# ktncktnc/diffusion-forcing-transformer

Hardware: AMD Instinct MI355X
Metric: denoised latent frames/sec, DFoT RE10K 8f & 200f rollout @1/2/4/8 GPU (higher is better)
Workload: dtype bf16

## Files before the change

diffusion-forcing-transformer_amd/backbone.py:

```python
from __future__ import annotations

import ctypes as C
import math
from typing import Dict, Optional, Sequence, Tuple

import torch
from torch import nn

from . import capi, ops


def _get(cfg, key, default=None):
    if isinstance(cfg, dict):
        return cfg.get(key, default)
    return getattr(cfg, key, default) if not hasattr(cfg, "get") else cfg.get(key, default)


class _Node(nn.Module):
    """Anonymous container so that dotted reference key names map onto a module tree."""


class UViT3DPose(nn.Module):
    def __init__(self, cfg, x_shape: Sequence[int], max_tokens: int, external_cond_dim: int = 0,
                 external_cond_type: str = "action", external_cond_num_classes: Optional[int] = None,
# ... 42 lines not shown
            self._register(name, tuple(shape[k] for k in range(ndim.value)))
            self._names.append(name)
        self._synced: Optional[Tuple] = None
        self._reserved = 0
        self._op_key: Optional[int] = None
        self._cond_key = None
        self._cond_refs = None
        self._cond_gen = None
        self._cond_flag = None
        self.cond_cache_stats = {"builds": 0, "identity_hits": 0, "content_hits": 0}
        self._train_names = None
        self._trainer = None
        self._trainer_sig = None
        self.live_frames = None
        self.fresh_frames = None
        self._fresh_key = None
        self._train_stamp = 0
        self._dropout_generator: Optional[torch.Generator] = None

    def _register(self, name: str, shape: Tuple[int, ...]) -> None:
        *path, leaf = name.split(".")
        node: nn.Module = self
        for part in path:
            if part not in node._modules:
                node.add_module(part, _Node())
            node = node._modules[part]
        t = torch.zeros(shape, dtype=torch.float32)
        if name in self._persistent_buffers:
            node.register_buffer(leaf, t, persistent=True)
        else:
# ... 228 lines not shown
            self._cond_refs = (external_cond, external_cond_mask)
            self._cond_gen = self.reserve_generation
        out = torch.empty_like(xf)
        live = self.live_frames
        if live is not None:
            if tuple(live.shape) != (b, self.temporal_length) or live.dtype != torch.uint8 or not live.is_contiguous():
                raise ValueError(f"live_frames must be a contiguous uint8 tensor of shape {(b, self.temporal_length)}")
            capi.require_device(dev, live_frames=live)
        fresh = self.fresh_frames
        if fresh is not None:
            if tuple(fresh.shape) != (b, self.temporal_length) or fresh.dtype != torch.uint8 or not fresh.is_contiguous():
                raise ValueError(f"fresh_frames must be a contiguous uint8 tensor of shape {(b, self.temporal_length)}")
            capi.require_device(dev, fresh_frames=fresh)
            if key != self._fresh_key:
                fresh = None
        capi.check(capi.lib.dfot_uvit_forward_cached_masks(self._handle, capi.ptr(xf, torch.float32, "x"),
                                                           capi.ptr(kf, torch.float32, "noise_levels"), capi.ptr(out), b,
                                                           capi.ptr(live, torch.uint8, "live_frames"),
                                                           capi.ptr(fresh, torch.uint8, "fresh_frames"), capi.stream_ptr()))
        self._fresh_key = key
        return out.to(x.dtype)

    def read_tap(self, name: str, channels: int, level: int, batch: int) -> torch.Tensor:
        r = self.x_shape[-1] // 2 // (2 ** level)
        out = torch.empty(batch * self.temporal_length, channels, r, r, device="cuda", dtype=torch.float32)
        capi.check(capi.lib.dfot_uvit_read_tap(self._handle, name.encode(), capi.ptr(out), out.numel(), capi.stream_ptr()))
        return out

    def __del__(self):
        try:
            if getattr(self, "_handle", None) and self._handle.value:
                capi.lib.dfot_uvit_destroy(self._handle)
                self._handle = C.c_void_p()
        except Exception:
# ... 2 lines not shown
```

diffusion-forcing-transformer_amd/capi.py:

```python
from __future__ import annotations

import ctypes as C
import os

_HERE = os.path.dirname(os.path.abspath(__file__))
LIB_PATH = os.environ.get("DFOT_LIB", os.path.join(_HERE, "libdfot_hip.so"))

OK, ERR_ARG, ERR_SHAPE, ERR_HIP, ERR_STATE, ERR_NAME = range(6)


class DfotError(RuntimeError):
    def __init__(self, code: int, message: str):
        super().__init__(f"libdfot_hip error {code}: {message}")
        self.code = code


class UViTConfig(C.Structure):
    _fields_ = [
        ("channels", C.c_int32 * 4), ("emb_channels", C.c_int32), ("num_updown_blocks", C.c_int32 * 3),
        ("num_mid_blocks", C.c_int32), ("num_heads", C.c_int32), ("in_channels", C.c_int32),
        ("resolution", C.c_int32), ("max_tokens", C.c_int32), ("cond_dim", C.c_int32), ("noise_dim", C.c_int32),
        ("rope_theta", C.c_float), ("eps", C.c_float),
    ]

# ... 53 lines not shown
    "dfot_uvit_num_params": (_I, [_P]),
    "dfot_uvit_param_name": (C.c_char_p, [_P, _I]),
    "dfot_uvit_param_shape": (_I, [_P, _I, C.POINTER(_L), C.POINTER(_I)]),
    "dfot_uvit_load_weight": (_I, [_P, C.c_char_p, _P, C.POINTER(_L), _I, _P]),
    "dfot_uvit_finalize": (_I, [_P, _P]),
    "dfot_uvit_reserve": (_I, [_P, _I]),
    "dfot_uvit_workspace_bytes": (C.c_size_t, [_P]),
    "dfot_uvit_set_option": (_I, [_P, C.c_char_p, _I]),
    "dfot_uvit_query": (_I, [_P, C.c_char_p, C.POINTER(C.c_double)]),
    "dfot_uvit_attn_timing": (_I, [_P, C.POINTER(C.c_double), C.POINTER(_L)]),
    "dfot_uvit_forward": (_I, [_P, _P, _P, _P, _P, _P, _I, _P]),
    "dfot_uvit_set_conditions": (_I, [_P, _P, _P, _I, _P]),
    "dfot_uvit_forward_cached": (_I, [_P, _P, _P, _P, _I, _P]),
    "dfot_uvit_forward_cached_live": (_I, [_P, _P, _P, _P, _I, _P, _P]),
    "dfot_uvit_forward_cached_masks": (_I, [_P, _P, _P, _P, _I, _P, _P, _P]),
    "dfot_uvit_read_tap": (_I, [_P, C.c_char_p, _P, C.c_size_t, _P]),
    "dfot_uvit3d_create": (_I, [C.POINTER(UViT3DConfig), C.POINTER(_P)]),
    "dfot_uvit3d_config_bytes": (_L, []),
    "dfot_uvit3d_forward": (_I, [_P, _P, _P, _P, _P, _P, _I, _P]),
    "dfot_uvit3d_forward_live": (_I, [_P, _P, _P, _P, _P, _P, _I, _P, _P]),
    "dfot_op_gn_film_silu": (_I, [_P, _P, _P, _P, _P, _P, _P, _P, _I, _I, _I, _I, _P]),
    "dfot_op_rms_film": (_I, [_P, _P, _P, _P, _P, _P, _L, _I, _I, _I, _F, _P]),
    "dfot_dit_create": (_I, [C.POINTER(DiTConfig), C.POINTER(_P)]),
    "dfot_dit_create_f": (_I, [C.POINTER(DiTConfigF), C.POINTER(_P)]),
    "dfot_dit_destroy": (_I, [_P]),
    "dfot_dit_num_params": (_I, [_P]),
    "dfot_dit_param_name": (C.c_char_p, [_P, _I]),
    "dfot_dit_param_shape": (_I, [_P, _I, C.POINTER(_L), C.POINTER(_I)]),
    "dfot_dit_load_weight": (_I, [_P, C.c_char_p, _P, C.POINTER(_L), _I, _P]),
    "dfot_dit_finalize": (_I, [_P, _P]),
# ... 163 lines not shown
```

diffusion-forcing-transformer_amd/csrc/kernels.h:

```cpp
#pragma once
#include "common.h"

namespace dfot {

int launch_noise_emb(const float* k, const float* freqs, const float* phases, const float* w1, const float* b1,
                     const float* w2, const float* b2, float* hidden, float* out, int bt, int ndim, int e, hipStream_t s);
int launch_uvit3d_emb(const float* k, const float* freqs, const float* phases, const float* w1, const float* b1, const float* w2,
                      const float* b2, const float* cond, const uint8_t* cond_mask, const float* a_w1, const float* a_b1,
                      const float* a_w2, const float* a_b2, float* out, int bt, int ndim, int cdim, int e, int tokens, hipStream_t s);
int launch_embed_input(const float* x, const float* w, const float* b, float* out, int bt, int res, int cin, int c0,
                       hipStream_t s);
int launch_cond_repack(const float* cond, bf16* a, int bt, int res, int cdim, int kpad, hipStream_t s);
int launch_emb_pyramid(const bf16* emb0, bf16* emb1, bf16* emb2, bf16* emb3, int bt, int r0, int e, hipStream_t s);
int launch_project_output(const float* x0, const float* w, const float* b, float* out, int bt, int res, int c0, int cout,
                          hipStream_t s, const uint8_t* live = nullptr);
int launch_gn_partial_f32(const float* x, float* partial, int bt, int pixels, int c, hipStream_t s);
int launch_gn_partial_bf16(const bf16* x, float* partial, int bt, int pixels, int c, hipStream_t s);
int launch_gn_finalize(const float* partial, float* stats, int bt, int nblk, int pixels, int c, float eps, hipStream_t s);
int gn_partial_blocks(int pixels);
int launch_gn_apply_silu(const float* x, const float* stats, const float* gamma, const float* beta, bf16* out, int bt,
                         int pixels, int c, hipStream_t s, const uint8_t* live = nullptr);
struct FilmChunk {
  const bf16* w;
  const float* b;
// ... 42 lines not shown
                    int img_w = 0, int sdy = 0, int sdx = 0, int all_taps = 0);
struct WgradPlan {
  int form, slices;
};
WgradPlan wgrad_plan(int m, int n, long rows, long max_slices);
int launch_wgrad_conv_taps(const bf16* dy, const bf16* x, float* out, int co, int ci, long pix, int slices, int img_h, int img_w, hipStream_t s);
int wgrad_conv_tiles(int co, int ci, int* target);
int launch_wgrad_nt_plan(const bf16* a, long lda, const bf16* b, long ldb, float* out, int m, int n, long rows, WgradPlan plan, hipStream_t s);
int launch_vloss_grad(const float* x, const float* noise, const float* v, const float* a, const float* sg, const float* coef, float* dv,
                      int batch, int tokens, long f, bool vspace, hipStream_t s);
int launch_sumsq(const float* x, long n, float* out, hipStream_t s);
int launch_adamw(float* p, const float* g, float* m, float* v, long n, float lr, float b1, float b2, float eps, float wd, int step,
                 const float* sumsq, float max_norm, float* ema, float ema_decay, hipStream_t s);
int launch_f32_to_bf16(const float* src, bf16* dst, long n, hipStream_t s);
int launch_bf16_to_f32(const bf16* src, float* dst, long n, hipStream_t s);
int launch_equal_bits(const void* a, const void* b, long bytes, int* differs, hipStream_t s);
int launch_pack_rows(const float* src, bf16* dst, const int* map, int rows, int k, int kpad, long ldd, int col0,
                     hipStream_t s);
int launch_pack_conv3(const float* src, bf16* dst, int co, int ci, hipStream_t s);
int launch_gather_f32(const float* src, float* dst, const int* map, int n, hipStream_t s);
int launch_nhwc_to_nchw(const float* src, float* dst, int bt, int p, int c, hipStream_t s);
int launch_bf16_nhwc_to_nchw(const bf16* src, float* dst, int bt, int p, int c, hipStream_t s);

struct AttnScratch {
  float* p = nullptr;
  size_t bytes = 0;
};
int launch_attention(const bf16* q, const bf16* k, const bf16* v, bf16* o, long ldo, int batch, int heads, int n, int d,
                     int variant, hipStream_t stream, AttnScratch* scratch = nullptr);
int launch_attention_v3(const bf16* q, const bf16* k, const bf16* v, bf16* o, long ldo, int batch, int heads, int n, bool nomax,
// ... 31 lines not shown
```

diffusion-forcing-transformer_amd/csrc/kernels.hip:

```cpp
#include "kernels.h"
#include "dfot_hip.h"

namespace dfot {

typedef __attribute__((ext_vector_type(4))) float float4v;
typedef __attribute__((ext_vector_type(2))) float float2v;

__device__ __forceinline__ float wave_sum(float v) {
#pragma unroll
  for (int o = 32; o > 0; o >>= 1) v += __shfl_xor(v, o);
  return v;
}

template <bool FOURIER>
__global__ __launch_bounds__(256) void noise_mlp_kernel(const float* __restrict__ in, const float* __restrict__ freqs,
                                                        const float* __restrict__ phases, const float* __restrict__ w,
                                                        const float* __restrict__ b, float* __restrict__ out, int kdim,
                                                        int e) {
  const int lane = threadIdx.x & 63, wave = threadIdx.x >> 6;
  const int row = blockIdx.x * 4 + wave;
  const int bt = blockIdx.y;
  if (row >= e) return;
  float acc = 0.f;
  for (int i = lane; i < kdim; i += 64) {
// ... 1293 lines not shown
  const bf16x8 v = reinterpret_cast<const bf16x8*>(s)[i];
  float4v a, b;
#pragma unroll
  for (int j = 0; j < 4; ++j) a[j] = bf2f(v[j]), b[j] = bf2f(v[4 + j]);
  reinterpret_cast<float4v*>(d)[2 * i] = a;
  reinterpret_cast<float4v*>(d)[2 * i + 1] = b;
}
static bool aligned16(const void* a, const void* b) { return (((uintptr_t)a | (uintptr_t)b) & 15) == 0; }
int launch_f32_to_bf16(const float* src, bf16* dst, long n, hipStream_t s) {
  const long n8 = aligned16(src, dst) ? n / 8 : 0;
  if (n8) hipLaunchKernelGGL(f32_to_bf16_kernel8, dim3(cdiv(n8, 256)), dim3(256), 0, s, src, dst, n8);
  if (n - 8 * n8) hipLaunchKernelGGL(f32_to_bf16_kernel, dim3(cdiv(n - 8 * n8, 256)), dim3(256), 0, s, src + 8 * n8, dst + 8 * n8, n - 8 * n8);
  DFOT_CHECK_HIP(hipGetLastError());
  return DFOT_OK;
}
int launch_bf16_to_f32(const bf16* src, float* dst, long n, hipStream_t s) {
  const long n8 = aligned16(src, dst) ? n / 8 : 0;
  if (n8) hipLaunchKernelGGL(bf16_to_f32_kernel8, dim3(cdiv(n8, 256)), dim3(256), 0, s, src, dst, n8);
  if (n - 8 * n8) hipLaunchKernelGGL(bf16_to_f32_kernel, dim3(cdiv(n - 8 * n8, 256)), dim3(256), 0, s, src + 8 * n8, dst + 8 * n8, n - 8 * n8);
  DFOT_CHECK_HIP(hipGetLastError());
  return DFOT_OK;
}

__global__ void pack_rows_kernel(const float* __restrict__ src, bf16* __restrict__ dst, const int* __restrict__ map, long total,
                                 int k, int kpad, long ldd, int col0) {
  const long i = (long)blockIdx.x * blockDim.x + threadIdx.x;
  if (i >= total) return;
  const int kk = (int)(i % kpad);
  const long r = i / kpad;
  const long sr = map ? map[r] : r;
// ... 207 lines not shown
```

diffusion-forcing-transformer_amd/csrc/uvit.hip:

```cpp
#include <algorithm>
#include <cmath>
#include <cstdarg>
#include <cstdlib>
#include <cstring>
#include <functional>
#include <map>
#include <string>
#include <vector>

#include "dfot_hip.h"
#include "gemm.h"
#include "kernels.h"

namespace dfot {

static thread_local char g_err[1024] = "";
void set_error(const char* fmt, ...) {
  va_list ap;
  va_start(ap, fmt);
  vsnprintf(g_err, sizeof(g_err), fmt, ap);
  va_end(ap);
}
const char* get_error() { return g_err; }

// ... 71 lines not shown
  int film_chunks = 0;
  uint8_t* cond_mask = nullptr;
  bool have_mask = false;
  int cond_batch = 0;
  int64_t cond_builds = 0;
  bf16 *acond = nullptr, *emb[4] = {nullptr, nullptr, nullptr, nullptr}, *s1 = nullptr, *hbf = nullptr,
       *cat = nullptr, *q = nullptr, *k = nullptr, *v = nullptr;
  AttnScratch attn_scratch;
  const float* pend_part = nullptr;
  float* out_part = nullptr;
  size_t out_part_elems = 0;
  const float* pend_bias = nullptr;
  int pend_lvl = 0, pend_c = 0, pend_slices = 2;
  long pend_m = 0;
  int last_batch = 0;
  const float* xin[4] = {nullptr, nullptr, nullptr, nullptr};
  bf16* XB[4] = {nullptr, nullptr, nullptr, nullptr};
  bool xin_bf[4] = {false, false, false, false};
  int gemm_variant = GEMM_AUTO;
  int attn_variant = 2;
  bool attn_force_safe = false;
  bool time_attn = false;
  std::vector<hipEvent_t> ev_start, ev_stop;
  size_t ev_used = 0;
};

namespace dfot {

template <typename T>
static int dev_alloc(dfot_uvit_s* h, T** out, size_t count, bool workspace = false) {
// ... 428 lines not shown
  g.A = h->s1; g.W = h->up_conv[l].w; g.M = bt * rr * rr; g.N = cout; g.K = 9 * cin; g.H = rr; g.Wd = rr; g.Cin = cin;
  g.zeros = h->zeros; g.bias = h->up_conv[l].b; g.out_f32 = h->tmp; g.ldo = cout;
  if (live && (rr * rr) % 256 == 0 && h->gemm_variant == GEMM_AUTO) g.live = live;
  if ((rc = conv_between_levels(h, g, s))) return rc;
  h->gn1_nblk = 0;
  if (!h->xin_bf[l]) {
    set_error("run_up: level %d stream is not in its bf16 buffer", l);
    return DFOT_ERR_STATE;
  }
  return launch_upsample_add_bf16(h->tmp, h->XB[l], h->XB[l], bt, rr, rr, cout, s, live);
}

}

static int forward_from_emb(dfot_uvit_s* h, const float* x, float* out, int batch, const uint8_t* live_frames, const uint8_t* fresh_frames,
                            hipStream_t s);

extern "C" {

const char* dfot_last_error(void) { return get_error(); }
int dfot_version(void) { return 1; }

int dfot_uvit_create(const dfot_uvit_config* cfg, dfot_uvit_t* out) {
  DFOT_REQUIRE(cfg && out, DFOT_ERR_ARG, "dfot_uvit_create: null argument");
  DFOT_REQUIRE(cfg->resolution % 16 == 0 && cfg->resolution >= 32, DFOT_ERR_SHAPE, "resolution %d must be a multiple of 16", cfg->resolution);
  DFOT_REQUIRE(cfg->emb_channels % 64 == 0, DFOT_ERR_SHAPE, "emb_channels %d must be a multiple of 64", cfg->emb_channels);
  DFOT_REQUIRE(cfg->in_channels <= 3 && cfg->cond_dim % 20 == 0, DFOT_ERR_SHAPE, "in_channels %d / cond_dim %d unsupported", cfg->in_channels, cfg->cond_dim);
  for (int l = 0; l < 4; ++l)
    DFOT_REQUIRE(cfg->channels[l] % 64 == 0, DFOT_ERR_SHAPE, "channels[%d]=%d must be a multiple of 64", l, cfg->channels[l]);
  DFOT_REQUIRE(cfg->channels[0] % 128 == 0 && cfg->channels[1] % 128 == 0, DFOT_ERR_SHAPE, "ResBlock channels must be multiples of 128");
  for (int l = 2; l < 4; ++l) {
// ... 180 lines not shown
      sv_off += (long)bt * 2 * c;
      return DFOT_OK;
    };
    for (int l = 0; l < 2; ++l) {
      for (ResW& w : h->down_res[l]) if ((rc = add(&w.fcache, &w.sv_off, w.w_film, w.b_film, w.c, l))) return rc;
      for (ResW& w : h->up_res[l]) if ((rc = add(&w.fcache, &w.sv_off, w.w_film, w.b_film, w.c, l))) return rc;
    }
    for (TrW& w : h->down_tr) if ((rc = add(&w.fcache, &w.sv_off, w.w_film, w.b_film, w.c, 2))) return rc;
    for (TrW& w : h->up_tr) if ((rc = add(&w.fcache, &w.sv_off, w.w_film, w.b_film, w.c, 2))) return rc;
    for (TrW& w : h->mid_tr) if ((rc = add(&w.fcache, &w.sv_off, w.w_film, w.b_film, w.c, 3))) return rc;
    if ((rc = dev_alloc(h, &h->sv, (size_t)sv_off, true))) return rc;
    if ((rc = dev_alloc(h, &h->film_table, table.size(), true))) return rc;
    DFOT_CHECK_HIP(hipMemcpy(h->film_table, table.data(), table.size() * sizeof(FilmChunk), hipMemcpyHostToDevice));
    h->film_chunks = (int)table.size();
    if ((rc = dev_alloc(h, &h->cond_mask, (size_t)max_batch, true))) return rc;
    h->cond_batch = 0;
  }
  if ((rc = dev_alloc(h, &h->cat, mc * 5, true))) return rc;
  if ((rc = dev_alloc(h, &h->q, mc, true))) return rc;
  if ((rc = dev_alloc(h, &h->k, mc, true))) return rc;
  if ((rc = dev_alloc(h, &h->v, mc, true))) return rc;
  {
    const size_t e2 = bt * pix[2] * h->ch[2], e3 = bt * pix[3] * h->ch[3];
    h->out_part_elems = 3 * (e2 > e3 ? e2 : e3);
    if ((rc = dev_alloc(h, &h->out_part, h->out_part_elems, true))) return rc;
  }
  {
    size_t need = 16;
    for (int b = 1; b <= max_batch; ++b)
      for (int l = 2; l < 4; ++l) need = std::max(need, attention_scratch_bytes(b, h->heads, h->T * h->r[l] * h->r[l], h->ch[l] / h->heads));
// ... 41 lines not shown
    set_error("set_option: unknown key '%s'", key);
    return DFOT_ERR_ARG;
  }
  return DFOT_OK;
}

int dfot_uvit_query(dfot_uvit_t h, const char* key, double* value) {
  DFOT_REQUIRE(h && key && value, DFOT_ERR_ARG, "query: null argument");
  DFOT_REQUIRE(h->finalized, DFOT_ERR_STATE, "query: weights not finalized");
  float bound = 0.f;
  for (const TrW& w : h->down_tr) bound = fmaxf(bound, w.score_bound);
  for (const TrW& w : h->up_tr) bound = fmaxf(bound, w.score_bound);
  if (!strcmp(key, "score_bound_l2")) *value = bound;
  else if (!strcmp(key, "attn_kernel_l2")) *value = (bound < 64.0f && !h->attn_force_safe) ? 14 : 5;
  else if (!strcmp(key, "cond_builds")) *value = (double)h->cond_builds;
  else {
    set_error("query: unknown key '%s'", key);
    return DFOT_ERR_ARG;
  }
  return DFOT_OK;
}

int dfot_uvit_set_conditions(dfot_uvit_t h, const float* external_cond, const uint8_t* external_cond_mask, int batch,
                             void* stream) {
  DFOT_REQUIRE(h, DFOT_ERR_ARG, "set_conditions: null handle");
  DFOT_REQUIRE(!h->posefree, DFOT_ERR_STATE, "set_conditions: a pose-free handle (dfot_uvit3d_create) has no pose caches; call dfot_uvit3d_forward");
  DFOT_REQUIRE(external_cond != nullptr, DFOT_ERR_ARG, "External condition (camera pose) is required for U-ViT3DPose model.");
  DFOT_REQUIRE(h->finalized, DFOT_ERR_STATE, "set_conditions: weights not finalized");
  DFOT_REQUIRE(batch > 0 && batch <= h->max_batch, DFOT_ERR_STATE, "set_conditions: batch %d exceeds reserved %d", batch, h->max_batch);
  hipStream_t s = (hipStream_t)stream;
// ... 28 lines not shown
  h->cond_batch = batch;
  return DFOT_OK;
}

int dfot_uvit_forward_cached(dfot_uvit_t h, const float* x, const float* noise_levels, float* out, int batch, void* stream) {
  return dfot_uvit_forward_cached_live(h, x, noise_levels, out, batch, nullptr, stream);
}

int dfot_uvit_forward_cached_live(dfot_uvit_t h, const float* x, const float* noise_levels, float* out, int batch, const uint8_t* live_frames,
                                  void* stream) {
  return dfot_uvit_forward_cached_masks(h, x, noise_levels, out, batch, live_frames, nullptr, stream);
}

int dfot_uvit_forward_cached_masks(dfot_uvit_t h, const float* x, const float* noise_levels, float* out, int batch, const uint8_t* live_frames,
                                   const uint8_t* fresh_frames, void* stream) {
  DFOT_REQUIRE(h && x && noise_levels && out, DFOT_ERR_ARG, "forward: null argument");
  DFOT_REQUIRE(!fresh_frames || h->last_batch == batch, DFOT_ERR_STATE,
               "forward: frozen frames need the previous forward of this handle to have run the same batch (%d, now %d)", h->last_batch, batch);
  DFOT_REQUIRE(!fresh_frames || live_frames, DFOT_ERR_ARG, "forward: frozen frames must also be dead frames (live_frames is null)");
  DFOT_REQUIRE(!h->posefree, DFOT_ERR_STATE, "forward_cached: a pose-free handle (dfot_uvit3d_create) runs through dfot_uvit3d_forward");
  DFOT_REQUIRE(h->finalized, DFOT_ERR_STATE, "forward: weights not finalized");
  DFOT_REQUIRE(batch > 0 && batch == h->cond_batch, DFOT_ERR_STATE,
               "forward_cached: batch %d does not match the cached conditions (%d)", batch, h->cond_batch);
  hipStream_t s = (hipStream_t)stream;
  const dfot_uvit_config& c = h->cfg;
  const int bt = batch * h->T, e = h->E;
  int rc = 0;
  if ((rc = launch_noise_emb(noise_levels, h->ne_freqs, h->ne_phases, h->ne_w1, h->ne_b1, h->ne_w2, h->ne_b2, h->nhid,
                             h->nemb, bt, c.noise_dim, e, s)))
    return rc;
  return forward_from_emb(h, x, out, batch, live_frames, fresh_frames, s);
}

}

static int forward_from_emb(dfot_uvit_s* h, const float* x, float* out, int batch, const uint8_t* live_frames, const uint8_t* fresh_frames,
                            hipStream_t s) {
  const dfot_uvit_config& c = h->cfg;
  const int bt = batch * h->T, e = h->E;
  int rc = 0;
  if ((rc = launch_film_vec(h->film_table, h->film_chunks, h->nemb, h->sv, bt, e, s))) return rc;
  if ((rc = launch_embed_input_bf16(x, h->ein_w, h->ein_b, h->XB[0], bt, c.resolution, c.in_channels, h->ch[0], s))) return rc;
  h->gn1_nblk = 0;
  for (int l = 0; l < 4; ++l) h->xin[l] = h->X[l];
  h->xin_bf[0] = true;
  h->xin_bf[1] = h->xin_bf[2] = h->xin_bf[3] = false;

  if (fresh_frames && (h->gemm_variant != GEMM_AUTO || (h->r[2] * h->r[2]) % 512 != 0)) fresh_frames = nullptr;
  for (int l = 0; l < 2; ++l) {
    for (const ResW& w : h->down_res[l])
      if ((rc = run_res_block(h, w, l, bt, s, fresh_frames))) return rc;
    if ((rc = run_down(h, l, bt, s, fresh_frames))) return rc;
  }
  h->pend_bias = nullptr;
  for (const TrW& w : h->down_tr)
    if ((rc = run_tr_block(h, w, 2, batch, s))) return rc;
  if ((rc = flush_pending(h, s))) return rc;
  if ((rc = run_down(h, 2, bt, s))) return rc;
  for (const TrW& w : h->mid_tr)
    if ((rc = run_tr_block(h, w, 3, batch, s))) return rc;
  if ((rc = flush_pending(h, s))) return rc;
  if ((rc = run_up(h, 2, bt, s))) return rc;
  for (const TrW& w : h->up_tr)
    if ((rc = run_tr_block(h, w, 2, batch, s))) return rc;
  if ((rc = flush_pending(h, s))) return rc;
  for (int l = 1; l >= 0; --l) {
    if ((rc = run_up(h, l, bt, s, live_frames))) return rc;
// ... 211 lines not shown
```

diffusion-forcing-transformer_amd/sampler.py:

```python
from __future__ import annotations

from dataclasses import dataclass, field
from typing import Callable, Dict, List, Optional, Tuple

import numpy as np
import torch

from . import capi, parallel
from .diffusion import DiffusionConfig, Schedule
from .guidance import HistoryGuidance


@dataclass
class SamplerConfig:
    x_shape: Tuple[int, int, int] = (3, 256, 256)
    max_tokens: int = 8
    diffusion: DiffusionConfig = field(default_factory=DiffusionConfig)
    scheduling_matrix: str = "full_sequence"
    is_full_sequence: bool = False
    prediction_guidance: Dict = field(default_factory=lambda: {"name": "conditional"})
    interpolation_guidance: Dict = field(default_factory=lambda: {"name": "conditional"})
    keyframe_density: Optional[float] = None
    sliding_context_len: Optional[int] = None
    interpolation_max_batch_size: Optional[int] = None
# ... 21 lines not shown
        self.schedule = Schedule(cfg.diffusion)
        self.noise_fn = noise_fn or device_noise_fn(clip=cfg.diffusion.clip_noise)
        self.timesteps = cfg.diffusion.timesteps
        self.sampling_timesteps = cfg.diffusion.sampling_timesteps
        self.max_tokens = cfg.max_tokens
        self.x_shape = tuple(cfg.x_shape)
        self.trace: List[dict] = []
        self.window_forwards = 0
        self.shard_windows = False
        self.branch_parallel = False
        self._branch_split_active = False
        self.device = "cuda"
        self.dry_run = False
        self.use_graph = True
        self.skip_frozen_frames = True
        self.skip_dead_frames = True
        self.graph_replays = 0
        self.graph_captures = 0
        self._graphs: Dict[tuple, dict] = {}
        self._graphs_generation = 0
        if cfg.diffusion.sampling_timesteps > cfg.diffusion.timesteps:
            raise ValueError("sampling_timesteps must be <= timesteps")

    @torch.no_grad()
    def _process_conditions(self, conditions: Optional[torch.Tensor], noise_levels=None) -> Optional[torch.Tensor]:
        if conditions is None:
            return None
        if conditions.shape[-1] != 16:
            raise ValueError(f"raw camera poses must have 16 values per frame, got {conditions.shape[-1]}")
        cfg = self.cfg
# ... 187 lines not shown
            qb = np.where(repl, qb_c, np.float32(0)).astype(np.float32)
            excl = None
            if plan.excluded is not None:
                excl = plan.excluded.reshape(bm, horizon)
                qa, qb = np.where(excl, np.float32(0), qa), np.where(excl, np.float32(1), qb)
            sa, s1, an, cn, keepf, sigma = sch.ddim_coef(lv, tl) if sch.is_ddim_sampling else sch.ddpm_coef(lv)
            sigma = np.where(keepf != 0, np.float32(0), sigma).astype(np.float32)
            tables = np.stack([qa, qb, sa, s1, an, cn, keepf, sch.model_level(lv)]).astype(np.float32)
            plans.append(dict(plan=plan, nfe=plan.nfe, bm=bm, need_noise=bool(repl.any()) or excl is not None, excl=excl, tables=tables,
                              sigma=sigma if bool((sigma != 0).any()) else None,
                              gen=(mask == 0).astype(np.uint8),
                              cmask=None if plan.cond_masked is None else np.tile(plan.cond_masked, batch_size)))
        if not plans:
            return (xs[:, :-padding] if padding > 0 else xs), None
        strict = bool(getattr(self.noise_fn, "strict_order", False))

        def draw_noise(p_):
            nfe, bm, need = p_["nfe"], p_["bm"], p_["need_noise"]
            noise = None
            if history_guidance.is_simple:
                if nfe == 2 and (need or strict):
                    drawn = self.noise_fn("q_sample", (batch_size, horizon, *x_shape))
                    noise = torch.zeros(batch_size, 2, horizon, *x_shape, device=dev, dtype=torch.float32)
                    noise[:, 0] = drawn.to(device=dev, dtype=torch.float32)
            else:
                g = p_["plan"].n_gen
                bh = bm // g
                if need or strict:
                    noise = self.noise_fn("q_sample", (bh, horizon, *x_shape)).to(device=dev, dtype=torch.float32)
                    if g > 1:
# ... 70 lines not shown
                for p_ in plans:
                    if p_.get("renoise"):
                        continue
                    lv = p_["plan"].levels.reshape(p_["bm"], horizon)
                    key = (lv == self.timesteps - 1).tobytes() + bytes([p_["nfe"]])
                    if key not in by_mask:
                        by_mask[key] = self._process_conditions(conditions.repeat_interleave(p_["nfe"], dim=0), lv)
                    p_["cond"] = by_mask[key]
            finally:
                self._interpolate_masked_poses = False
        fresh_dev = torch.from_numpy(np.concatenate([a.ravel() for a in self._fresh_flags(plans, batch_size, horizon)])).cuda()
        foff = 0
        for p_ in plans:
            p_["fresh_dev"] = fresh_dev[foff:foff + p_["bm"] * horizon].view(p_["bm"], horizon)
            foff += p_["bm"] * horizon
        xs = xs.contiguous()
        s = capi.stream_ptr
        branch_cache: Dict[tuple, tuple] = {}

        skip_dead = self.skip_dead_frames and hasattr(self.model, "live_frames")
        skip_frozen = skip_dead and self.skip_frozen_frames and hasattr(self.model, "fresh_frames")

        def step(p_, xs, noise, tables, gen_dev, xs_next=None, live_dev=None, fresh_dev=None):
            nonlocal cond_rep, cond_nfe
            nfe, bm = p_["nfe"], p_["bm"]
            x_in = torch.empty(bm, horizon, *x_shape, device="cuda", dtype=torch.float32)
            capi.check(capi.lib.dfot_hg_prepare(capi.ptr(xs), capi.ptr(noise), capi.ptr(tables[0]), capi.ptr(tables[1]),
                                                capi.ptr(x_in), batch_size, nfe, horizon, f, s()))
            if cond_full is not None and cond_nfe != nfe:
                cond_rep = cond_full if nfe == 1 else cond_full.repeat_interleave(nfe, dim=0)
                cond_nfe = nfe
            if "cond" in p_:
                cond_rep = p_["cond"]
            lvl = tables[7] if cfg.diffusion.is_continuous else tables[7].to(torch.int32)
            world, rank = parallel.world_info()
            if nfe in split_nfe:
                hb = rank % nfe
                key = (id(cond_rep), id(p_["cmask_dev"]), hb)
# ... 7 lines not shown
                if skip_dead:
                    self.model.live_frames = gen_dev
                try:
                    v = parallel.exchange_branches(self.model(x_h, l_h, c_h, m_h), nfe)
                    self.branch_exchanges = getattr(self, "branch_exchanges", 0) + 1
                finally:
                    if skip_dead:
                        self.model.live_frames = None
            elif rg > 0:
                v = self._reconstruction_guided_v(x_in, lvl, cond_rep, p_["cmask_dev"], tables, gen_dev, rg_ctx, rg, nfe)
            else:
                if skip_dead:
                    self.model.live_frames = live_dev if live_dev is not None else p_["live_dev"]
                if skip_frozen:
                    self.model.fresh_frames = fresh_dev if fresh_dev is not None else p_["fresh_dev"]
                try:
                    v = self.model(x_in, lvl, cond_rep, p_["cmask_dev"])
                finally:
                    if skip_dead:
                        self.model.live_frames = None
                    if skip_frozen:
                        self.model.fresh_frames = None
            step_noise = None
            if strict or p_["sigma"] is not None:
                step_noise = self.noise_fn("ddim", (bm, horizon, *x_shape))
            if xs_next is None:
                xs_next = torch.empty_like(xs)
            compose = capi.lib.dfot_ddim_compose_tokw if p_["tokw"] else capi.lib.dfot_ddim_compose
            capi.check(compose(capi.ptr(xs), capi.ptr(x_in), capi.ptr(v), capi.ptr(tables[2]),
                                                  capi.ptr(tables[3]), capi.ptr(tables[4]), capi.ptr(tables[5]),
                                                  capi.ptr(tables[6]), capi.ptr(p_["weights_dev"]), capi.ptr(gen_dev),
                                                  capi.ptr(xs_next), batch_size, nfe, horizon, f, s()))
            if p_["sigma"] is not None:
                nz = step_noise.to(device="cuda", dtype=torch.float32).clamp(-cfg.diffusion.clip_noise, cfg.diffusion.clip_noise).contiguous()
                capi.check(capi.lib.dfot_ddim_noise(capi.ptr(nz), capi.ptr(p_["sigma_dev"]), capi.ptr(p_["weights_dev"]), capi.ptr(gen_dev),
                                                    capi.ptr(xs_next), batch_size, nfe, horizon, f, int(p_["tokw"]), s()))
            return xs_next
# ... 74 lines not shown
            if p_.get("renoise"):
                out.append(fresh)
                prev = None
                continue
            if (prev is not None and prev["bm"] == p_["bm"] and prev["nfe"] == p_["nfe"] and prev.get("cond") is p_.get("cond")
                    and ((prev["cmask"] is None and p_["cmask"] is None)
                         or (prev["cmask"] is not None and p_["cmask"] is not None and np.array_equal(prev["cmask"], p_["cmask"])))):
                a, b = prev["tables"], p_["tables"]
                same_in = (a[0] == 1) & (a[1] == 0) & (b[0] == 1) & (b[1] == 0) & (a[7] == b[7])
                untouched = np.repeat(prev["gen"].reshape(batch_size, horizon) == 0, p_["nfe"], axis=0)
                fresh = np.where(same_in & untouched, 0, 1).astype(np.uint8)
            out.append(fresh)
            prev = p_
        return out

    def _run_steps_graph(self, plans, xs, draw_noise, step, flat_dev, gens_dev, horizon):
        p0 = plans[0]
        bm, n_steps, nfe = p0["bm"], len(plans), p0["nfe"]
        need_noise = any(p_["need_noise"] for p_ in plans)
        self.model.reserve(bm)
        if hasattr(self.model, "sync_weights"):
            self.model.sync_weights()
        gen = getattr(self.model, "reserve_generation", 0)
        if gen != self._graphs_generation:
            self._graphs.clear()
            self._graphs_generation = gen
        cond_src = p0.get("cond_src")
        key = (bm, n_steps, nfe, horizon, tuple(xs.shape), need_noise, None if p0["cmask"] is None else p0["cmask"].tobytes(),
               id(self.model), None if cond_src is None else (tuple(cond_src.shape), cond_src.dtype))
        ent = self._graphs.get(key)
        if ent is None:
            ent = dict(tables=torch.empty(n_steps, 8, bm, horizon, device="cuda", dtype=torch.float32),
                       gens=torch.empty_like(gens_dev), weights=torch.empty_like(p0["weights_dev"]),
                       lives=torch.empty(n_steps, bm, horizon, device="cuda", dtype=torch.uint8),
                       fresh=torch.empty(n_steps, bm, horizon, device="cuda", dtype=torch.uint8),
                       noise=torch.empty(n_steps, bm, *xs.shape[1:], device="cuda") if need_noise else None,
                       xs=torch.empty_like(xs), out=None, graph=None,
                       cond=None if cond_src is None else torch.empty_like(cond_src))
        ent["tables"].copy_(flat_dev.view(n_steps, 8, bm, horizon))
        ent["gens"].copy_(gens_dev)
        ent["lives"].copy_(gens_dev if nfe == 1 else gens_dev.repeat_interleave(nfe, dim=1))
        ent["fresh"].copy_(torch.stack([p_["fresh_dev"] for p_ in plans]))
        ent["weights"].copy_(p0["weights_dev"])
        if need_noise:
            for i, p_ in enumerate(plans):
                if p_["need_noise"]:
                    ent["noise"][i].copy_(draw_noise(p_))
                else:
                    ent["noise"][i].zero_()
        p_static = dict(p0, weights_dev=ent["weights"])
        if cond_src is not None:
            ent["cond"].copy_(cond_src)
            p_static["cond"] = ent["cond"]
        ent["xs"].copy_(step(p_static, xs, None if not need_noise else ent["noise"][0], ent["tables"][0], ent["gens"][0], live_dev=ent["lives"][0],
                            fresh_dev=ent["fresh"][0]))
        if ent["graph"] is None:
            torch.cuda.synchronize()
            graph = torch.cuda.CUDAGraph()
            with torch.cuda.graph(graph, capture_error_mode="thread_local"):
                x = ent["xs"]
                for i in range(1, n_steps):
                    x = step(p_static, x, ent["noise"][i] if need_noise else None, ent["tables"][i], ent["gens"][i], live_dev=ent["lives"][i],
                             fresh_dev=ent["fresh"][i])
                ent["out"] = x
            ent["graph"] = graph
            if len(self._graphs) >= 4:
                self._graphs.pop(next(iter(self._graphs)))
            self._graphs[key] = ent
            self.graph_captures += 1
        ent["graph"].replay()
        self.graph_replays += n_steps - 1
        return ent["out"].clone()

    @torch.no_grad()
    def _predict_sequence(self, context: torch.Tensor, length: Optional[int] = None,
                          conditions: Optional[torch.Tensor] = None, history_guidance: Optional[HistoryGuidance] = None,
                          sliding_context_len: Optional[int] = None, **_) -> Tuple[torch.Tensor, None]:
        mt = self.max_tokens
# ... 206 lines not shown
```

include/dfot_hip.h:

```cpp
#ifndef DFOT_HIP_H_
#define DFOT_HIP_H_

#include <stddef.h>
#include <stdint.h>

#ifdef __cplusplus
extern "C" {
#endif

enum {
  DFOT_OK = 0,
  DFOT_ERR_ARG = 1,
  DFOT_ERR_SHAPE = 2,
  DFOT_ERR_HIP = 3,
  DFOT_ERR_STATE = 4,
  DFOT_ERR_NAME = 5
};

typedef struct dfot_uvit_s* dfot_uvit_t;

typedef struct {
  int32_t channels[4];
  int32_t emb_channels;
  int32_t num_updown_blocks[3];
// ... 23 lines not shown
size_t dfot_uvit_workspace_bytes(dfot_uvit_t h);
int dfot_uvit_set_option(dfot_uvit_t h, const char* key, int value);
int dfot_uvit_query(dfot_uvit_t h, const char* key, double* value);
int dfot_uvit_attn_timing(dfot_uvit_t h, double* total_ms, int64_t* launches);

int dfot_uvit_forward(dfot_uvit_t h, const float* x, const float* noise_levels, const float* external_cond,
                      const uint8_t* external_cond_mask, float* out, int batch, void* stream);
int dfot_uvit_set_conditions(dfot_uvit_t h, const float* external_cond, const uint8_t* external_cond_mask, int batch,
                             void* stream);
int dfot_uvit_forward_cached(dfot_uvit_t h, const float* x, const float* noise_levels, float* out, int batch,
                             void* stream);
int dfot_uvit_forward_cached_live(dfot_uvit_t h, const float* x, const float* noise_levels, float* out, int batch,
                                  const uint8_t* live_frames, void* stream);
int dfot_uvit_forward_cached_masks(dfot_uvit_t h, const float* x, const float* noise_levels, float* out, int batch,
                                   const uint8_t* live_frames, const uint8_t* fresh_frames, void* stream);
int dfot_uvit_read_tap(dfot_uvit_t h, const char* name, float* out, size_t capacity_floats, void* stream);

typedef struct {
  int32_t channels[4];
  int32_t emb_channels;
  int32_t num_updown_blocks[3];
  int32_t num_mid_blocks;
  int32_t num_heads;
  int32_t in_channels;
  int32_t resolution;
  int32_t max_tokens;
  int32_t cond_dim;
  int32_t noise_dim;
  float rope_theta;
  float eps;
// ... 252 lines not shown
```

Before: 10.36.

## Skip down-path compute for frames shared across guidance branches and copy results

Detects frames whose input, noise level and condition mask are identical across the NFE guidance branches of a batch. For those frames it runs the down-path res blocks only for the first branch, then copies the activations into the other branches with a new row-copy kernel. This removes redundant convolution and GEMM work in the encoder stages under history guidance. In exchange it adds host-side flag computation, a mask kernel, several copy launches per forward and more state threaded through graph capture.

```diff
diff --git a/diffusion-forcing-transformer_amd/backbone.py b/diffusion-forcing-transformer_amd/backbone.py
--- a/diffusion-forcing-transformer_amd/backbone.py
+++ b/diffusion-forcing-transformer_amd/backbone.py
@@ -4,6 +4,7 @@
 import math
 from typing import Dict, Optional, Sequence, Tuple
 
+import numpy as np
 import torch
 from torch import nn
 
@@ -80,6 +81,10 @@
         self._trainer_sig = None
         self.live_frames = None
         self.fresh_frames = None
+        self.shared_frames = None
+        self.shared_frames_host = None
+        self.share_group = 0
+        self._ones_flags = None
         self._fresh_key = None
         self._train_stamp = 0
         self._dropout_generator: Optional[torch.Generator] = None
@@ -338,10 +343,33 @@
             capi.require_device(dev, fresh_frames=fresh)
             if key != self._fresh_key:
                 fresh = None
-        capi.check(capi.lib.dfot_uvit_forward_cached_masks(self._handle, capi.ptr(xf, torch.float32, "x"),
-                                                           capi.ptr(kf, torch.float32, "noise_levels"), capi.ptr(out), b,
-                                                           capi.ptr(live, torch.uint8, "live_frames"),
-                                                           capi.ptr(fresh, torch.uint8, "fresh_frames"), capi.stream_ptr()))
+        shared = self.shared_frames if live is not None else None
+        if shared is not None:
+            host = self.shared_frames_host
+            if tuple(shared.shape) != (b, self.temporal_length) or shared.dtype != torch.uint8 or not shared.is_contiguous():
+                raise ValueError(f"shared_frames must be a contiguous uint8 tensor of shape {(b, self.temporal_length)}")
+            if host is None or tuple(host.shape) != (b, self.temporal_length) or host.dtype != np.uint8:
+                raise ValueError(f"shared_frames_host must be the uint8 numpy copy of shared_frames, shape {(b, self.temporal_length)}")
+            capi.require_device(dev, shared_frames=shared)
+            if fresh is None:
+                if self._ones_flags is None or self._ones_flags.shape != shared.shape or self._ones_flags.device != dev:
+                    self._ones_flags = None if torch.cuda.is_current_stream_capturing() else torch.ones_like(shared)
+                fresh = self._ones_flags
+            if fresh is None:
+                shared = None
+        if shared is not None:
+            capi.check(capi.lib.dfot_uvit_shared_frames_host(self._handle, np.ascontiguousarray(host).tobytes(), host.size))
+            capi.check(capi.lib.dfot_uvit_forward_cached_shared(self._handle, capi.ptr(xf, torch.float32, "x"),
+                                                                capi.ptr(kf, torch.float32, "noise_levels"), capi.ptr(out), b,
+                                                                capi.ptr(live, torch.uint8, "live_frames"),
+                                                                capi.ptr(fresh, torch.uint8, "fresh_frames"),
+                                                                capi.ptr(shared, torch.uint8, "shared_frames"), int(self.share_group),
+                                                                capi.stream_ptr()))
+        else:
+            capi.check(capi.lib.dfot_uvit_forward_cached_masks(self._handle, capi.ptr(xf, torch.float32, "x"),
+                                                               capi.ptr(kf, torch.float32, "noise_levels"), capi.ptr(out), b,
+                                                               capi.ptr(live, torch.uint8, "live_frames"),
+                                                               capi.ptr(fresh, torch.uint8, "fresh_frames"), capi.stream_ptr()))
         self._fresh_key = key
         return out.to(x.dtype)
 
diff --git a/diffusion-forcing-transformer_amd/capi.py b/diffusion-forcing-transformer_amd/capi.py
--- a/diffusion-forcing-transformer_amd/capi.py
+++ b/diffusion-forcing-transformer_amd/capi.py
@@ -91,6 +91,8 @@
     "dfot_uvit_forward_cached": (_I, [_P, _P, _P, _P, _I, _P]),
     "dfot_uvit_forward_cached_live": (_I, [_P, _P, _P, _P, _I, _P, _P]),
     "dfot_uvit_forward_cached_masks": (_I, [_P, _P, _P, _P, _I, _P, _P, _P]),
+    "dfot_uvit_shared_frames_host": (_I, [_P, C.c_char_p, _I]),
+    "dfot_uvit_forward_cached_shared": (_I, [_P, _P, _P, _P, _I, _P, _P, _P, _I, _P]),
     "dfot_uvit_read_tap": (_I, [_P, C.c_char_p, _P, C.c_size_t, _P]),
     "dfot_uvit3d_create": (_I, [C.POINTER(UViT3DConfig), C.POINTER(_P)]),
     "dfot_uvit3d_config_bytes": (_L, []),
diff --git a/diffusion-forcing-transformer_amd/csrc/kernels.h b/diffusion-forcing-transformer_amd/csrc/kernels.h
--- a/diffusion-forcing-transformer_amd/csrc/kernels.h
+++ b/diffusion-forcing-transformer_amd/csrc/kernels.h
@@ -80,6 +80,9 @@
                  const float* sumsq, float max_norm, float* ema, float ema_decay, hipStream_t s);
 int launch_f32_to_bf16(const float* src, bf16* dst, long n, hipStream_t s);
 int launch_bf16_to_f32(const bf16* src, float* dst, long n, hipStream_t s);
+int launch_shared_masks(const uint8_t* fresh, const uint8_t* shared, const uint8_t* live, uint8_t* down_mask, uint8_t* copy_mask, int bt, int tokens,
+                        int group, bool use_fresh, hipStream_t s);
+int launch_copy_shared_rows(void* base, long bytes_per_image, const uint8_t* copy_mask, int bt, int tokens, int group, hipStream_t s);
 int launch_equal_bits(const void* a, const void* b, long bytes, int* differs, hipStream_t s);
 int launch_pack_rows(const float* src, bf16* dst, const int* map, int rows, int k, int kpad, long ldd, int col0,
                      hipStream_t s);
diff --git a/diffusion-forcing-transformer_amd/csrc/kernels.hip b/diffusion-forcing-transformer_amd/csrc/kernels.hip
--- a/diffusion-forcing-transformer_amd/csrc/kernels.hip
+++ b/diffusion-forcing-transformer_amd/csrc/kernels.hip
@@ -1331,6 +1331,47 @@
   DFOT_CHECK_HIP(hipGetLastError());
   return DFOT_OK;
 }
+__global__ void shared_masks_kernel(const uint8_t* __restrict__ fresh, const uint8_t* __restrict__ shared, const uint8_t* __restrict__ live,
+                                    uint8_t* __restrict__ down_mask, uint8_t* __restrict__ copy_mask, int bt, int tokens, int group, int use_fresh) {
+  const int i = blockIdx.x * blockDim.x + threadIdx.x;
+  if (i >= bt) return;
+  const int br = (i / tokens) % group, src = i - br * tokens;
+  const bool fr = !use_fresh || fresh[i], fr_src = !use_fresh || fresh[src];
+  const bool cp = shared[i] && br != 0 && (fr_src || !live[i]);
+  copy_mask[i] = cp ? 1 : 0;
+  down_mask[i] = (fr && !cp) ? 1 : 0;
+}
+int launch_shared_masks(const uint8_t* fresh, const uint8_t* shared, const uint8_t* live, uint8_t* down_mask, uint8_t* copy_mask, int bt, int tokens,
+                        int group, bool use_fresh, hipStream_t s) {
+  DFOT_REQUIRE(fresh && shared && live && down_mask && copy_mask, DFOT_ERR_ARG, "shared_masks: null argument");
+  DFOT_REQUIRE(bt > 0 && tokens > 0 && group >= 2 && bt % (tokens * group) == 0, DFOT_ERR_SHAPE, "shared_masks: %d images, %d tokens, group %d", bt,
+               tokens, group);
+  hipLaunchKernelGGL(shared_masks_kernel, dim3(cdiv(bt, 256)), dim3(256), 0, s, fresh, shared, live, down_mask, copy_mask, bt, tokens, group,
+                     use_fresh ? 1 : 0);
+  DFOT_CHECK_HIP(hipGetLastError());
+  return DFOT_OK;
+}
+__global__ void copy_shared_rows_kernel(float4v* __restrict__ base, long img16, const uint8_t* __restrict__ copy_mask, int tokens, int group) {
+  const int img = blockIdx.y;
+  if (!copy_mask[img]) return;
+  const int br = (img / tokens) % group;
+  float4v* dst = base + (long)img * img16;
+  const float4v* src = base + (long)(img - br * tokens) * img16;
+  for (long i = (long)blockIdx.x * blockDim.x + threadIdx.x; i < img16; i += (long)gridDim.x * blockDim.x) dst[i] = src[i];
+}
+int launch_copy_shared_rows(void* base, long bytes_per_image, const uint8_t* copy_mask, int bt, int tokens, int group, hipStream_t s) {
+  DFOT_REQUIRE(base && copy_mask, DFOT_ERR_ARG, "copy_shared_rows: null argument");
+  DFOT_REQUIRE(bt > 0 && bt < 65536 && tokens > 0 && group >= 2 && bt % (tokens * group) == 0, DFOT_ERR_SHAPE,
+               "copy_shared_rows: %d images, %d tokens, group %d", bt, tokens, group);
+  DFOT_REQUIRE(bytes_per_image > 0 && bytes_per_image % 16 == 0 && ((uintptr_t)base & 15) == 0, DFOT_ERR_SHAPE,
+               "copy_shared_rows: %ld bytes per image / the base pointer must be multiples of 16", bytes_per_image);
+  const long img16 = bytes_per_image / 16;
+  const int gx = img16 < 128 * 256 ? cdiv(img16, 256) : 128;
+  hipLaunchKernelGGL(copy_shared_rows_kernel, dim3(gx, bt), dim3(256), 0, s, (float4v*)base, img16, copy_mask, tokens, group);
+  DFOT_CHECK_HIP(hipGetLastError());
+  return DFOT_OK;
+}
+
 int launch_bf16_to_f32(const bf16* src, float* dst, long n, hipStream_t s) {
   const long n8 = aligned16(src, dst) ? n / 8 : 0;
   if (n8) hipLaunchKernelGGL(bf16_to_f32_kernel8, dim3(cdiv(n8, 256)), dim3(256), 0, s, src, dst, n8);
diff --git a/diffusion-forcing-transformer_amd/csrc/uvit.hip b/diffusion-forcing-transformer_amd/csrc/uvit.hip
--- a/diffusion-forcing-transformer_amd/csrc/uvit.hip
+++ b/diffusion-forcing-transformer_amd/csrc/uvit.hip
@@ -109,6 +109,9 @@
   int pend_lvl = 0, pend_c = 0, pend_slices = 2;
   long pend_m = 0;
   int last_batch = 0;
+  uint8_t *down_mask = nullptr, *copy_mask = nullptr;
+  std::vector<uint8_t> shared_host;
+  int64_t shared_skipped = 0;
   const float* xin[4] = {nullptr, nullptr, nullptr, nullptr};
   bf16* XB[4] = {nullptr, nullptr, nullptr, nullptr};
   bool xin_bf[4] = {false, false, false, false};
@@ -567,7 +570,7 @@
 }
 
 static int forward_from_emb(dfot_uvit_s* h, const float* x, float* out, int batch, const uint8_t* live_frames, const uint8_t* fresh_frames,
-                            hipStream_t s);
+                            hipStream_t s, const uint8_t* shared_frames = nullptr, int group = 0, bool use_fresh = true);
 
 extern "C" {
 
@@ -778,6 +781,8 @@
     DFOT_CHECK_HIP(hipMemcpy(h->film_table, table.data(), table.size() * sizeof(FilmChunk), hipMemcpyHostToDevice));
     h->film_chunks = (int)table.size();
     if ((rc = dev_alloc(h, &h->cond_mask, (size_t)max_batch, true))) return rc;
+    if ((rc = dev_alloc(h, &h->down_mask, bt, true))) return rc;
+    if ((rc = dev_alloc(h, &h->copy_mask, bt, true))) return rc;
     h->cond_batch = 0;
   }
   if ((rc = dev_alloc(h, &h->cat, mc * 5, true))) return rc;
@@ -849,6 +854,7 @@
   if (!strcmp(key, "score_bound_l2")) *value = bound;
   else if (!strcmp(key, "attn_kernel_l2")) *value = (bound < 64.0f && !h->attn_force_safe) ? 14 : 5;
   else if (!strcmp(key, "cond_builds")) *value = (double)h->cond_builds;
+  else if (!strcmp(key, "shared_frames_skipped")) *value = (double)h->shared_skipped;
   else {
     set_error("query: unknown key '%s'", key);
     return DFOT_ERR_ARG;
@@ -907,8 +913,32 @@
 
 int dfot_uvit_forward_cached_masks(dfot_uvit_t h, const float* x, const float* noise_levels, float* out, int batch, const uint8_t* live_frames,
                                    const uint8_t* fresh_frames, void* stream) {
+  return dfot_uvit_forward_cached_shared(h, x, noise_levels, out, batch, live_frames, fresh_frames, nullptr, 0, stream);
+}
+
+int dfot_uvit_shared_frames_host(dfot_uvit_t h, const uint8_t* flags, int count) {
+  DFOT_REQUIRE(h && count >= 0 && (flags || count == 0), DFOT_ERR_ARG, "shared_frames_host: bad argument");
+  h->shared_host.assign(flags, flags + count);
+  return DFOT_OK;
+}
+
+int dfot_uvit_forward_cached_shared(dfot_uvit_t h, const float* x, const float* noise_levels, float* out, int batch, const uint8_t* live_frames,
+                                    const uint8_t* fresh_frames, const uint8_t* shared_frames, int group, void* stream) {
   DFOT_REQUIRE(h && x && noise_levels && out, DFOT_ERR_ARG, "forward: null argument");
-  DFOT_REQUIRE(!fresh_frames || h->last_batch == batch, DFOT_ERR_STATE,
+  bool use_fresh = true;
+  if (shared_frames) {
+    DFOT_REQUIRE(live_frames && fresh_frames, DFOT_ERR_ARG, "forward: shared frames need live_frames and fresh_frames");
+    DFOT_REQUIRE(group >= 2 && batch > 0 && batch % group == 0, DFOT_ERR_ARG, "forward: shared frames need a group >= 2 that divides the batch (group %d, batch %d)",
+                 group, batch);
+    DFOT_REQUIRE((long)h->shared_host.size() == (long)batch * h->T, DFOT_ERR_ARG,
+                 "forward: shared frames need the host copy of the flags (dfot_uvit_shared_frames_host: %ld bytes, expected %ld)",
+                 (long)h->shared_host.size(), (long)batch * h->T);
+    for (int b = 0; b < batch; b += group)
+      for (int t = 0; t < h->T; ++t)
+        DFOT_REQUIRE(!h->shared_host[(size_t)b * h->T + t], DFOT_ERR_ARG, "forward: frame %d of row %d, the first row of its group, is flagged as shared", t, b);
+    use_fresh = h->last_batch == batch;
+  }
+  DFOT_REQUIRE(!fresh_frames || !use_fresh || h->last_batch == batch, DFOT_ERR_STATE,
                "forward: frozen frames need the previous forward of this handle to have run the same batch (%d, now %d)", h->last_batch, batch);
   DFOT_REQUIRE(!fresh_frames || live_frames, DFOT_ERR_ARG, "forward: frozen frames must also be dead frames (live_frames is null)");
   DFOT_REQUIRE(!h->posefree, DFOT_ERR_STATE, "forward_cached: a pose-free handle (dfot_uvit3d_create) runs through dfot_uvit3d_forward");
@@ -922,13 +952,13 @@
   if ((rc = launch_noise_emb(noise_levels, h->ne_freqs, h->ne_phases, h->ne_w1, h->ne_b1, h->ne_w2, h->ne_b2, h->nhid,
                              h->nemb, bt, c.noise_dim, e, s)))
     return rc;
-  return forward_from_emb(h, x, out, batch, live_frames, fresh_frames, s);
+  return forward_from_emb(h, x, out, batch, live_frames, fresh_frames, s, shared_frames, group, use_fresh);
 }
 
 }
 
 static int forward_from_emb(dfot_uvit_s* h, const float* x, float* out, int batch, const uint8_t* live_frames, const uint8_t* fresh_frames,
-                            hipStream_t s) {
+                            hipStream_t s, const uint8_t* shared_frames, int group, bool use_fresh) {
   const dfot_uvit_config& c = h->cfg;
   const int bt = batch * h->T, e = h->E;
   int rc = 0;
@@ -939,11 +969,25 @@
   h->xin_bf[0] = true;
   h->xin_bf[1] = h->xin_bf[2] = h->xin_bf[3] = false;
 
-  if (fresh_frames && (h->gemm_variant != GEMM_AUTO || (h->r[2] * h->r[2]) % 512 != 0)) fresh_frames = nullptr;
+  if (fresh_frames && (h->gemm_variant != GEMM_AUTO || (h->r[2] * h->r[2]) % 512 != 0)) fresh_frames = shared_frames = nullptr;
+  h->shared_skipped = 0;
+  const uint8_t* down_mask = fresh_frames;
+  if (shared_frames) {
+    if ((rc = launch_shared_masks(fresh_frames, shared_frames, live_frames, h->down_mask, h->copy_mask, bt, h->T, group, use_fresh, s))) return rc;
+    down_mask = h->down_mask;
+    for (uint8_t f : h->shared_host) h->shared_skipped += f != 0;
+  }
   for (int l = 0; l < 2; ++l) {
     for (const ResW& w : h->down_res[l])
-      if ((rc = run_res_block(h, w, l, bt, s, fresh_frames))) return rc;
-    if ((rc = run_down(h, l, bt, s, fresh_frames))) return rc;
+      if ((rc = run_res_block(h, w, l, bt, s, down_mask))) return rc;
+    if ((rc = run_down(h, l, bt, s, down_mask))) return rc;
+  }
+  if (shared_frames) {
+    const long px0 = (long)h->r[0] * h->r[0], px1 = (long)h->r[1] * h->r[1], px2 = (long)h->r[2] * h->r[2];
+    if ((rc = launch_copy_shared_rows(h->XB[0], px0 * h->ch[0] * (long)sizeof(bf16), h->copy_mask, bt, h->T, group, s))) return rc;
+    if ((rc = launch_copy_shared_rows(h->HSA[0], px1 * h->ch[1] * (long)sizeof(float), h->copy_mask, bt, h->T, group, s))) return rc;
+    if ((rc = launch_copy_shared_rows(h->XB[1], px1 * h->ch[1] * (long)sizeof(bf16), h->copy_mask, bt, h->T, group, s))) return rc;
+    if ((rc = launch_copy_shared_rows(h->HSA[1], px2 * h->ch[2] * (long)sizeof(float), h->copy_mask, bt, h->T, group, s))) return rc;
   }
   h->pend_bias = nullptr;
   for (const TrW& w : h->down_tr)
diff --git a/diffusion-forcing-transformer_amd/sampler.py b/diffusion-forcing-transformer_amd/sampler.py
--- a/diffusion-forcing-transformer_amd/sampler.py
+++ b/diffusion-forcing-transformer_amd/sampler.py
@@ -59,6 +59,7 @@
         self.dry_run = False
         self.use_graph = True
         self.skip_frozen_frames = True
+        self.skip_shared_frames = True
         self.skip_dead_frames = True
         self.graph_replays = 0
         self.graph_captures = 0
@@ -276,6 +277,9 @@
         if not plans:
             return (xs[:, :-padding] if padding > 0 else xs), None
         strict = bool(getattr(self.noise_fn, "strict_order", False))
+        for p_ in plans:
+            p_["pose_interp"] = pose_interp
+        shared_np = self._shared_flags(plans, batch_size, horizon)
 
         def draw_noise(p_):
             nfe, bm, need = p_["nfe"], p_["bm"], p_["need_noise"]
@@ -376,14 +380,22 @@
         for p_ in plans:
             p_["fresh_dev"] = fresh_dev[foff:foff + p_["bm"] * horizon].view(p_["bm"], horizon)
             foff += p_["bm"] * horizon
+        shared_dev = torch.from_numpy(np.concatenate([a.ravel() for a in shared_np])).cuda()
+        foff = 0
+        for p_, sh in zip(plans, shared_np):
+            if sh.any():
+                p_["shared_host"] = sh
+                p_["shared_dev"] = shared_dev[foff:foff + p_["bm"] * horizon].view(p_["bm"], horizon)
+            foff += p_["bm"] * horizon
         xs = xs.contiguous()
         s = capi.stream_ptr
         branch_cache: Dict[tuple, tuple] = {}
 
         skip_dead = self.skip_dead_frames and hasattr(self.model, "live_frames")
         skip_frozen = skip_dead and self.skip_frozen_frames and hasattr(self.model, "fresh_frames")
-
-        def step(p_, xs, noise, tables, gen_dev, xs_next=None, live_dev=None, fresh_dev=None):
+        skip_shared = skip_dead and self.skip_shared_frames and hasattr(self.model, "shared_frames")
+
+        def step(p_, xs, noise, tables, gen_dev, xs_next=None, live_dev=None, fresh_dev=None, shared=None):
             nonlocal cond_rep, cond_nfe
             nfe, bm = p_["nfe"], p_["bm"]
             x_in = torch.empty(bm, horizon, *x_shape, device="cuda", dtype=torch.float32)
@@ -421,6 +433,10 @@
                     self.model.live_frames = live_dev if live_dev is not None else p_["live_dev"]
                 if skip_frozen:
                     self.model.fresh_frames = fresh_dev if fresh_dev is not None else p_["fresh_dev"]
+                if shared is None and "shared_dev" in p_:
+                    shared = (p_["shared_dev"], p_["shared_host"])
+                if skip_shared and shared is not None:
+                    self.model.shared_frames, self.model.shared_frames_host, self.model.share_group = shared[0], shared[1], nfe
                 try:
                     v = self.model(x_in, lvl, cond_rep, p_["cmask_dev"])
                 finally:
@@ -428,6 +444,8 @@
                         self.model.live_frames = None
                     if skip_frozen:
                         self.model.fresh_frames = None
+                    if skip_shared:
+                        self.model.shared_frames, self.model.shared_frames_host, self.model.share_group = None, None, 0
             step_noise = None
             if strict or p_["sigma"] is not None:
                 step_noise = self.noise_fn("ddim", (bm, horizon, *x_shape))
@@ -532,6 +550,24 @@
             prev = p_
         return out
 
+    @staticmethod
+    def _shared_flags(plans, batch_size: int, horizon: int):
+        out = []
+        for p_ in plans:
+            nfe, bm = p_["nfe"], p_["bm"]
+            shared = np.zeros((bm, horizon), np.uint8)
+            if not p_.get("renoise") and nfe > 1 and not p_.get("pose_interp") and "cond" not in p_:
+                t = p_["tables"].reshape(8, batch_size, nfe, horizon)
+                qa, qb, lvl = t[0], t[1], t[7]
+                same = (qa == qa[:, :1]) & (qb == 0) & (qb[:, :1] == 0) & (lvl == lvl[:, :1])
+                if p_["cmask"] is not None:
+                    cm = np.asarray(p_["cmask"]).reshape(batch_size, nfe)
+                    same &= (cm == cm[:, :1])[:, :, None]
+                same[:, 0] = False
+                shared = same.reshape(bm, horizon).astype(np.uint8)
+            out.append(shared)
+        return out
+
     def _run_steps_graph(self, plans, xs, draw_noise, step, flat_dev, gens_dev, horizon):
         p0 = plans[0]
         bm, n_steps, nfe = p0["bm"], len(plans), p0["nfe"]
@@ -545,13 +581,14 @@
             self._graphs_generation = gen
         cond_src = p0.get("cond_src")
         key = (bm, n_steps, nfe, horizon, tuple(xs.shape), need_noise, None if p0["cmask"] is None else p0["cmask"].tobytes(),
-               id(self.model), None if cond_src is None else (tuple(cond_src.shape), cond_src.dtype))
+               id(self.model), None if cond_src is None else (tuple(cond_src.shape), cond_src.dtype), self.skip_shared_frames)
         ent = self._graphs.get(key)
         if ent is None:
             ent = dict(tables=torch.empty(n_steps, 8, bm, horizon, device="cuda", dtype=torch.float32),
                        gens=torch.empty_like(gens_dev), weights=torch.empty_like(p0["weights_dev"]),
                        lives=torch.empty(n_steps, bm, horizon, device="cuda", dtype=torch.uint8),
                        fresh=torch.empty(n_steps, bm, horizon, device="cuda", dtype=torch.uint8),
+                       shared=torch.empty(n_steps, bm, horizon, device="cuda", dtype=torch.uint8),
                        noise=torch.empty(n_steps, bm, *xs.shape[1:], device="cuda") if need_noise else None,
                        xs=torch.empty_like(xs), out=None, graph=None,
                        cond=None if cond_src is None else torch.empty_like(cond_src))
@@ -559,6 +596,10 @@
         ent["gens"].copy_(gens_dev)
         ent["lives"].copy_(gens_dev if nfe == 1 else gens_dev.repeat_interleave(nfe, dim=1))
         ent["fresh"].copy_(torch.stack([p_["fresh_dev"] for p_ in plans]))
+        share = any("shared_dev" in p_ for p_ in plans)
+        shared_host = [p_.get("shared_host", np.zeros((bm, horizon), np.uint8)) for p_ in plans]
+        ent["shared"].copy_(torch.from_numpy(np.stack(shared_host)))
+        shared_of = lambda i: (ent["shared"][i], shared_host[i]) if share else None
         ent["weights"].copy_(p0["weights_dev"])
         if need_noise:
             for i, p_ in enumerate(plans):
@@ -571,7 +612,7 @@
             ent["cond"].copy_(cond_src)
             p_static["cond"] = ent["cond"]
         ent["xs"].copy_(step(p_static, xs, None if not need_noise else ent["noise"][0], ent["tables"][0], ent["gens"][0], live_dev=ent["lives"][0],
-                            fresh_dev=ent["fresh"][0]))
+                            fresh_dev=ent["fresh"][0], shared=shared_of(0)))
         if ent["graph"] is None:
             torch.cuda.synchronize()
             graph = torch.cuda.CUDAGraph()
@@ -579,7 +620,7 @@
                 x = ent["xs"]
                 for i in range(1, n_steps):
                     x = step(p_static, x, ent["noise"][i] if need_noise else None, ent["tables"][i], ent["gens"][i], live_dev=ent["lives"][i],
-                             fresh_dev=ent["fresh"][i])
+                             fresh_dev=ent["fresh"][i], shared=shared_of(i))
                 ent["out"] = x
             ent["graph"] = graph
             if len(self._graphs) >= 4:
diff --git a/include/dfot_hip.h b/include/dfot_hip.h
--- a/include/dfot_hip.h
+++ b/include/dfot_hip.h
@@ -61,6 +61,10 @@
                                   const uint8_t* live_frames, void* stream);
 int dfot_uvit_forward_cached_masks(dfot_uvit_t h, const float* x, const float* noise_levels, float* out, int batch,
                                    const uint8_t* live_frames, const uint8_t* fresh_frames, void* stream);
+int dfot_uvit_shared_frames_host(dfot_uvit_t h, const uint8_t* flags, int count);
+int dfot_uvit_forward_cached_shared(dfot_uvit_t h, const float* x, const float* noise_levels, float* out, int batch,
+                                    const uint8_t* live_frames, const uint8_t* fresh_frames, const uint8_t* shared_frames, int group,
+                                    void* stream);
 int dfot_uvit_read_tap(dfot_uvit_t h, const char* name, float* out, size_t capacity_floats, void* stream);
 
 typedef struct {
```

Result: no change. 10.35 (-0.1%).
